# czbiohub-sf/biahub

Hardware: AMD Instinct MI355X
Metric: voxels/s for deskew+10-iter R-L deconv, 2048^2x512 f32 (higher is better)
Workload: dtype f32

## Files before the change

biahub_amd/build.py:

```python

from __future__ import annotations

import os
import subprocess
import sys
from concurrent.futures import ThreadPoolExecutor
from pathlib import Path

PKG = Path(__file__).resolve().parent
CSRC = PKG / "csrc"
INCLUDE = PKG.parent / "include"
LIB = PKG / "libbhcore.so"
SOURCES = ["pyramid.hip", "fftconv_col.hip", "fftconv_xtile.hip", "fftconv_xw.hip", "fftconv_colreg.hip", "deskew.hip", "stitch.hip", "stitch_pcc.hip", "affine.hip", "fftconv.hip", "context.hip", "fill.hip", "deconv.hip", "spline.hip", "copy.hip", "regmetric.hip", "flatfield.hip", "psf.hip", "binning.hip", "codec.hip", "lz4.hip", "zstd.hip", "mask.hip", "invtf.hip", "host_deskew.hip"]
ARCH = "gfx950"


def _hipcc() -> str:
    for cand in (os.environ.get("HIPCC"), "/opt/rocm/bin/hipcc", "hipcc"):
        if cand and (os.path.isabs(cand) and os.path.exists(cand) or not os.path.isabs(cand)):
            return cand
    return "hipcc"


_FC = ("fftconv.hpp", "fftconv_dev.hpp")
INCLUDES = {"fftconv.hip": _FC, "fftconv_col.hip": _FC, "fftconv_xtile.hip": _FC + ("fftconv_xpass.inc",), "fftconv_xw.hip": _FC + ("fftconv_xw.inc", "fftconv_x3.inc"),
            "fftconv_colreg.hip": _FC + ("fftconv_xw.inc", "fftconv_colw.inc", "fftconv_colz.inc", "fftconv_colz3.inc", "fftconv_zdirect.inc"),
            "deconv.hip": ("fftconv.hpp",), "invtf.hip": ("fftconv.hpp",), "affine.hip": ("affine_zwalk.inc", "affine_zoblique.inc"),
            "deskew.hip": ("deskew_geom.hpp", "deskew_rows.inc"), "host_deskew.hip": ("deskew_geom.hpp",), "zstd.hip": ("zstd_frame.inc", "zstd_block.inc")}


def needs_build() -> bool:
    if not LIB.exists():
        return True
    t = LIB.stat().st_mtime
    deps = [CSRC / s for s in SOURCES] + [CSRC / "common.hpp", INCLUDE / "bhcore.h"] + [CSRC / i for v in INCLUDES.values() for i in v]
    return any(d.stat().st_mtime > t for d in deps)


def build(force: bool = False, verbose: bool = True) -> Path:
    if not force and not needs_build():
        return LIB
    objdir = PKG / "build"
    objdir.mkdir(exist_ok=True)
    flags = ["-O3", f"--offload-arch={ARCH}", "-fPIC", "-std=c++17", f"-I{INCLUDE}", f"-I{CSRC}",
             "-Wall", "-Wno-unused-function"]

    def compile_one(src: str) -> Path:
# ... 26 lines not shown
```

biahub_amd/csrc/fftconv.hip:

```cpp
#include "fftconv_dev.hpp"

#include <mutex>

namespace bh {

static int x_tile_rows(int64_t X) { return X / 2 > 1024 ? 8 : BH_FC_XR; }

bool fftconv_supported_ex(int64_t Z, int64_t Y, int64_t X, bool radix3) {
    auto pow2 = [](int64_t v) { return v > 0 && (v & (v - 1)) == 0; };
    auto ok = [&](int64_t v) { return pow2(v) || (radix3 && ((v % 3 == 0 && pow2(v / 3)) || (v % 5 == 0 && pow2(v / 5)))); };
    if (!ok(Z) || !ok(Y) || !ok(X)) return false;
    if (X < 64 || X > 3072) return false;
    if (!pow2(X) && X / 2 / (X % 3 == 0 ? 3 : 5) < 32) return false;
    if (X / 4 > (X / 2 > 1024 ? BH_FC_XNT8 : BH_FC_XNT)) return false;
    if (Y < 2 * 16 || Y / 2 > 2048) return false;
    if (Z < 4 || Z > 2048) return false;
    const int xr = x_tile_rows(X);
    if ((Y % xr) != 0) return false;
    if (!pow2(Z) && Z / (Z % 3 == 0 ? 3 : 5) < 8) return false;
    if (!pow2(Y) && Y / 2 / (Y % 3 == 0 ? 3 : 5) < 16) return false;
    const int M = (int)X / 2, Lm = pow2(X) ? M : (X % 3 == 0 ? M / 3 : M / 5);
    const size_t xlds = (size_t)(M + 1) * (xr + 1) * 8 + (size_t)twiddle_count(Lm) * 8 + (size_t)M * 8 + (Lm != M ? (size_t)(M / Lm - 1) * Lm * 8 : 0);
    return xlds <= 160 * 1024;
}
// ... 301 lines not shown
    else
        hipLaunchKernelGGL(inverse_filter_rows_kernel<false>, dim3(grid), dim3(256), pl.d.XP * sizeof(cf), ctx->stream, tf, filt,
                           pl.d, reg, (float)(2.0 / V), bf16 ? 1 : 0, xcol);
    BH_CHECK_HIP(hipGetLastError());
    return BH_OK;
}

bool fftconv_fuses_normalisation(const ConvPlan& pl) { return pl.xw; }

int fftconv_apply_staged_filter(bh_ctx* ctx, const ConvPlan& pl, const float* in, const void* filt, bool bf16, cf* spec,
                                float* out, const double* norm_mean) {
    if (norm_mean) {
        BH_REQUIRE(pl.xw, "internal: fused normalisation needs the wave-private X passes");
        BH_TRY(launch_xw(ctx, pl, false, 0, in, spec, nullptr, nullptr, 0.f, false, norm_mean));
    } else
    BH_TRY(launch_x(ctx, pl, false, 0, in, spec, nullptr, nullptr, 0.f));
    BH_TRY(launch_col(ctx, pl, COL_FWD, false, spec, nullptr, 1.f));
    BH_TRY(launch_col(ctx, pl, bf16 ? COL_CONV16 : COL_CONV, true, spec, reinterpret_cast<const cf*>(filt), 1.f));
    BH_TRY(launch_col(ctx, pl, COL_INV, false, spec, nullptr, 1.f));
    BH_TRY(launch_x(ctx, pl, true, XE_STORE, nullptr, spec, out, nullptr, 0.f));
    return BH_OK;
}

int fftconv_richardson_lucy(bh_ctx* ctx, const ConvPlan& pl, const float* d, const cf* otf, bool otf_real, int zr, bool zreal, cf* spec,
                            int iterations, float eps, float* est) {
    if (iterations <= 0) return BH_OK;
    BH_TRY(launch_x(ctx, pl, false, 0, d, spec, est, nullptr, 0.f));
    for (int it = 0; it < iterations; ++it) {
        BH_TRY(launch_col(ctx, pl, COL_FWD, false, spec, nullptr, 1.f));
        BH_TRY(launch_rl_z(ctx, pl, false, otf_real, zr, zreal, spec, otf));
        BH_TRY(launch_col(ctx, pl, COL_INV, false, spec, nullptr, 1.f));
        BH_TRY(launch_x(ctx, pl, true, XE_RATIO, nullptr, spec, nullptr, d, eps, true));
        BH_TRY(launch_col(ctx, pl, COL_FWD, false, spec, nullptr, 1.f));
        BH_TRY(launch_rl_z(ctx, pl, true, otf_real, zr, zreal, spec, otf));
        BH_TRY(launch_col(ctx, pl, COL_INV, false, spec, nullptr, 1.f));
        BH_TRY(launch_x(ctx, pl, true, XE_UPDATE, nullptr, spec, est, est, eps, it + 1 < iterations));
    }
    return BH_OK;
}

int fftconv_tune_spectrum(bh_ctx* ctx, const ConvPlan& pl, float* est, size_t bytes, cf** spec) {
    const double V = (double)pl.d.Z * pl.d.Y * pl.d.X;
    const bool tune = env_int("BH_FC_TUNE_ALLOC", !(dev_alloc_is_shuffled() && dev_block_is_vmm(*spec))) != 0;
    if (!pl.xw || V < (double)(1u << 28) || !tune) return BH_OK;
    hipEvent_t e0, e1;
    BH_CHECK_HIP(hipEventCreate(&e0));
    BH_CHECK_HIP(hipEventCreate(&e1));
    auto audition = [&](cf* s, float* ms) -> int {
        for (int rep = 0; rep < 2; ++rep) {
            BH_CHECK_HIP(hipEventRecord(e0, ctx->stream));
            BH_TRY(launch_x(ctx, pl, true, XE_UPDATE, nullptr, s, est, est, 1e-6f, true));
            BH_CHECK_HIP(hipEventRecord(e1, ctx->stream));
            BH_CHECK_HIP(hipEventSynchronize(e1));
            BH_CHECK_HIP(hipEventElapsedTime(ms, e0, e1));
        }
        return BH_OK;
    };
    constexpr int NC = 5;
// ... 37 lines not shown
    BH_TRY(launch_col(ctx, pl, COL_FWD, false, spec, nullptr, 1.f));
    BH_TRY(launch_rl_z(ctx, pl, true, otf_real, zr, zreal, spec, otf));
    BH_TRY(launch_col(ctx, pl, COL_INV, false, spec, nullptr, 1.f));
    BH_TRY(launch_x(ctx, pl, true, XE_STORE, nullptr, spec, corr_p, nullptr, 0.f));
    return BH_OK;
}

bool fftconv_rl_wrap_supported(const ConvPlan& pl, const int64_t N[3], const int64_t K[3], const int64_t P[3]) {
    return pl.xw && N[1] == P[1] && K[2] <= 256 && getenv("BH_RL_NOWRAP") == nullptr;
}

int fftconv_richardson_lucy_wrap(bh_ctx* ctx, const ConvPlan& pl, const float* d_p, const cf* otf, bool otf_real, int zr, bool zreal, cf* spec_a,
                                 cf* spec_b, float* est_a, float* est_b, const int64_t N[3], const int64_t K[3], int iterations,
                                 float eps, float* out) {
    const int64_t P[3] = {pl.d.Z, pl.d.Y, pl.d.X};
    xw::Params::Wrap we[3], wr[3];
    for (int a = 0; a < 3; ++a) {
        const bool padded = P[a] != N[a];
        const int lo = padded ? (int)(K[a] - 1 - K[a] / 2) : 0, hi = padded ? (int)(K[a] / 2) : 0;
        we[a] = xw::Params::Wrap{(int)N[a], lo, lo, hi};
        wr[a] = xw::Params::Wrap{(int)N[a], lo, hi, lo};
    }
    float *cur = est_a, *nxt = est_b;
    BH_TRY(launch_x(ctx, pl, false, 0, d_p, spec_a, cur, nullptr, 0.f));
    for (int it = 0; it < iterations; ++it) {
        BH_TRY(launch_col(ctx, pl, COL_FWD, false, spec_a, nullptr, 1.f));
        BH_TRY(launch_rl_z(ctx, pl, false, otf_real, zr, zreal, spec_a, otf));
        BH_TRY(launch_col(ctx, pl, COL_INV, false, spec_a, nullptr, 1.f));
        BH_TRY(launch_xw_wrap(ctx, pl, xw::FUSED_RATIO_WRAP, spec_a, spec_b, nullptr, d_p, eps, wr[0], wr[2]));
        BH_TRY(launch_col(ctx, pl, COL_FWD, false, spec_b, nullptr, 1.f));
        BH_TRY(launch_rl_z(ctx, pl, true, otf_real, zr, zreal, spec_b, otf));
        BH_TRY(launch_col(ctx, pl, COL_INV, false, spec_b, nullptr, 1.f));
        if (it + 1 == iterations) {
            BH_TRY(launch_xw_wrap(ctx, pl, xw::INV_UPDATE_CROP, spec_b, nullptr, out, cur, eps, we[0], we[2]));
        } else {
            BH_TRY(launch_xw_wrap(ctx, pl, xw::FUSED_UPDATE_WRAP, spec_b, spec_a, nxt, cur, eps, we[0], we[2]));
            std::swap(cur, nxt);
        }
    }
    return BH_OK;
}

int fftconv_forward(bh_ctx* ctx, const ConvPlan& pl, const float* in, cf* spec) {
    BH_TRY(launch_x(ctx, pl, false, 0, in, spec, nullptr, nullptr, 0.f));
    BH_TRY(launch_col(ctx, pl, COL_FWD, false, spec, nullptr, 1.f));
    BH_TRY(launch_col(ctx, pl, COL_FWD, true, spec, nullptr, 1.f));
    return BH_OK;
}
int fftconv_inverse(bh_ctx* ctx, const ConvPlan& pl, cf* spec, float* out) {
    BH_TRY(launch_col(ctx, pl, COL_INV, true, spec, nullptr, 1.f));
    BH_TRY(launch_col(ctx, pl, COL_INV, false, spec, nullptr, 1.f));
    BH_TRY(launch_x(ctx, pl, true, XE_STORE, nullptr, spec, out, nullptr, 0.f));
    return BH_OK;
}

bool fftconv_pcc_peak_only(const ConvPlan& pl) { return pl.xw && !pl.x3 && getenv("BH_PCC_NO_FUSED_PEAK") == nullptr; }
int fftconv_pcc_apply(bh_ctx* ctx, const ConvPlan& pl, const float* img, cf* fixed, bool fixed_is_mov, bool roll, cf* s2, int norm,
// ... 33 lines not shown
```

biahub_amd/csrc/fftconv_colw.inc:

```
namespace colw {

#ifndef BH_COLW_NT
#define BH_COLW_NT 512
#endif
constexpr int NT = BH_COLW_NT;
constexpr int TILE_CF = 32 * NT;

template <int LOGN>
struct Geo {
    static constexpr int N = 1 << LOGN;
    static constexpr int W = TILE_CF / N;
    static constexpr int CPN = W / 2;
    static constexpr int N16 = N / 16, NQ = N / 256;
    static constexpr int LOWBITS = LOGN - 8;
    static constexpr int RC = 1 << LOWBITS;
    static constexpr int TILE_F4 = N * CPN + (N >> 5) * 8;
    static constexpr int NTA = 15 * N16, NTB = 15 * NQ;
    static constexpr size_t LDS_BYTES = (size_t)TILE_F4 * 16 + (size_t)(NTA + NTB) * 8;
};

template <int LOGN>
__host__ __device__ __forceinline__ constexpr int f4addr(int row, int cp) {
    return row * Geo<LOGN>::CPN + (row >> 5) * 8 + cp;
}

template <int LOGN>
__host__ __device__ __forceinline__ constexpr int row_a(int rest, int r) { return r * Geo<LOGN>::N16 + rest; }
template <int LOGN>
__host__ __device__ __forceinline__ constexpr int row_b(int rest, int r) {
// ... 93 lines not shown
    constexpr int DLOAD = LOAD_A ? 0 : DSPEC;
    constexpr int DSTORE = (MODE == COL_FWD || MODE == COL_FWD_SCALE) ? DSPEC : 0;
    extern __shared__ __attribute__((aligned(16))) unsigned char smem[];
    float4* tile = reinterpret_cast<float4*>(smem);
    cf* ta = reinterpret_cast<cf*>(smem + (size_t)G::TILE_F4 * 16);
    cf* tb = ta + G::NTA;
    const int tid = threadIdx.x;
    for (int i = tid; i < G::NTA + G::NTB; i += NT) ta[i] = p.tw[i];
    __syncthreads();
    const int cp = tid % G::CPN;
    const int ncoltiles = p.ncoltiles, nsub = p.nsub, XP = p.XP;
    const long outer_stride = p.outer_stride, sub_stride = p.sub_stride, row_stride = p.row_stride;
    const int ntiles = p.nouter * ncoltiles;
    auto tile_base = [=](int tt) -> long {
        const int ou = tt / ncoltiles;
        const int ct = tt - ou * ncoltiles;
        return (long)(ou / nsub) * outer_stride + (long)(ou % nsub) * sub_stride + (long)ct * G::W + 2 * cp;
    };
    const int rs = (int)row_stride;
    float4 pre[16];
    auto load_rows = [&](int tt, int rest) {
        const cf* src = p.S + tile_base(tt);
#pragma unroll
        for (int r = 0; r < 16; ++r) pre[r] = *reinterpret_cast<const float4*>(src + row_of<LOGN, DLOAD>(rest, r) * rs);
    };
    const int rest0 = tid / G::CPN;
    const int tstep = (int)gridDim.x;
    int t = (int)blockIdx.x;
    if (t < ntiles) load_rows(t, rest0);
    for (; t < ntiles; t += tstep) {
        const int rest = xw::opaque_i(rest0);
        const long base = tile_base(t);
        const int tn = t + tstep < ntiles ? t + tstep : t;
        cf x0[16], x1[16];
#pragma unroll
        for (int r = 0; r < 16; ++r) {
            x0[r] = make_float2(pre[r].x, pre[r].y);
            x1[r] = make_float2(pre[r].z, pre[r].w);
        }
        if (MODE == COL_INV) {
            load_rows(tn, rest);
            inverse<LOGN>(x0, x1, tile, ta, tb, rest, cp);
        } else if (!HAS_OTF) {
            load_rows(tn, rest);
            forward<LOGN>(x0, x1, tile, ta, tb, rest, cp);
            if (MODE == COL_FWD_SCALE) {
#pragma unroll
// ... 22 lines not shown
#pragma unroll
            for (int r = 0; r < 16; ++r) {
                const cf a0 = x0[r], a1 = x1[r];
                if (MODE == COL_FILTER) {
                    x0[r] = make_float2(a0.x * o[r].x, a0.y * o[r].y);
                    x1[r] = make_float2(a1.x * o[r].z, a1.y * o[r].w);
                } else if (MODE == COL_CORR) {
                    x0[r] = cmulc(a0, make_float2(o[r].x, o[r].y));
                    x1[r] = cmulc(a1, make_float2(o[r].z, o[r].w));
                } else {
                    x0[r] = cmul(a0, make_float2(o[r].x, o[r].y));
                    x1[r] = cmul(a1, make_float2(o[r].z, o[r].w));
                }
            }
            asm volatile("" ::: "memory");
            load_rows(tn, rest);
            __syncthreads();
            inverse<LOGN>(x0, x1, tile, ta, tb, rest, cp);
        }
        const bool col_ok = ((t % ncoltiles) * G::W + 2 * cp) < XP;
        if (col_ok) {
#pragma unroll
            for (int r = 0; r < 16; ++r)
                *reinterpret_cast<float4*>(p.S + base + row_of<LOGN, DSTORE>(rest, r) * rs) =
                    make_float4(x0[r].x, x0[r].y, x1[r].x, x1[r].y);
        }
        __syncthreads();
    }
}

template <int LOGN>
static void make_tables(std::vector<cf>& tab) {
    using G = Geo<LOGN>;
    tab.assign(G::NTA + G::NTB, make_float2(0.f, 0.f));
    for (int k = 1; k < 16; ++k) {
        for (int q = 0; q < G::N16; ++q) {
            const double a = -2.0 * M_PI * (double)q * k / (double)G::N;
            tab[(size_t)(k - 1) * G::N16 + q] = make_float2((float)std::cos(a), (float)std::sin(a));
        }
        for (int q = 0; q < G::NQ; ++q) {
            const double a = -2.0 * M_PI * (double)q * k / (double)G::N16;
            tab[G::NTA + (size_t)(k - 1) * G::NQ + q] = make_float2((float)std::cos(a), (float)std::sin(a));
        }
    }
}

}
```

biahub_amd/csrc/fftconv_dev.hpp:

```cpp
#pragma once
#include "fftconv.hpp"

#include <cmath>
#include <cstdio>
#include <cstdlib>
#include <utility>
#include <vector>

namespace bh {

#ifndef BH_FC_NT
#define BH_FC_NT 1024
#endif
constexpr int FC_NT = BH_FC_NT;
constexpr int FC_TILE = 16384;
#ifndef BH_FC_XR
#define BH_FC_XR 16
#endif
#ifndef BH_FC_XNT
#define BH_FC_XNT BH_FC_NT
#endif
#ifndef BH_FC_XNT8
#define BH_FC_XNT8 768
#endif
// ... 399 lines not shown
    float eps;
};

namespace xw {

enum Mode { FWD = 0, INV_STORE = 1, INV_RATIO = 2, INV_UPDATE = 3, FUSED_RATIO = 4, FUSED_UPDATE = 5, FUSED_RATIO_WRAP = 6, FUSED_UPDATE_WRAP = 7,
            INV_UPDATE_CROP = 8, INV_ARGMAX = 9 };

struct Params {
    const float* in;
    cf* S;
    float* out;
    const float* aux;
    const cf* tab;
    const cf* twy;
    int Z, Y, XP;
    float eps;
    const double* norm_mean;
    double* rowsum;
    cf* S_out;
    struct Wrap {
        int n, off, mlo, mhi;
    } wz, wx;
};

}


inline int ilog2(long v) {
    int l = 0;
    while ((1l << l) < v) ++l;
    return l;
}

inline bool env_off(const char* name) {
    const char* v = getenv(name);
    return v && atoi(v) == 0;
}
inline int env_int(const char* name, int dflt) {
    const char* v = getenv(name);
    return v ? atoi(v) : dflt;
}

template <typename K, typename P>
int launch_lds(bh_ctx* ctx, K kern, int grid, int threads, size_t lds, const P& p) {
    BH_CHECK_HIP(hipFuncSetAttribute(reinterpret_cast<const void*>(kern), hipFuncAttributeMaxDynamicSharedMemorySize, (int)lds));
    hipLaunchKernelGGL(kern, dim3(grid), dim3(threads), lds, ctx->stream, p);
    BH_CHECK_HIP(hipGetLastError());
    return BH_OK;
}

int launch_col_pass(bh_ctx* ctx, ColParams p, int mode);
int launch_col(bh_ctx* ctx, const ConvPlan& pl, int mode, bool zaxis, cf* S, const cf* otf, float scale, int pcc_norm = 0,
               int pcc_swap = 0, cf* otf_out = nullptr);
int launch_rl_z(bh_ctx* ctx, const ConvPlan& pl, bool corr, bool otf_real, int zr, bool zreal, cf* S, const cf* otf);
bool colw_tables(int64_t n, std::vector<cf>& tab);
bool colz_tables(const ConvDims& d, std::vector<cf>& tab);
bool colz3_tables(const ConvDims& d, std::vector<cf>& tab);
int launch_x_tile(bh_ctx* ctx, const ConvPlan& pl, bool inverse, int epi, const float* in, cf* S, float* out, const float* aux,
                  float eps, bool fuse_fwd);
void xw_tables(int64_t X, std::vector<cf>& tab, std::vector<int>& col);
int launch_xw(bh_ctx* ctx, const ConvPlan& pl, bool inverse, int epi, const float* in, cf* S, float* out, const float* aux,
              float eps, bool fuse_fwd, const double* norm_mean = nullptr);
int launch_xw_argmax(bh_ctx* ctx, const ConvPlan& pl, cf* S, ArgMax* partial, int* npartial);
int launch_xw_wrap(bh_ctx* ctx, const ConvPlan& pl, int mode, const cf* S_in, cf* S_out, float* out, const float* aux, float eps,
                   xw::Params::Wrap wz, xw::Params::Wrap wx);

}
```

biahub_amd/csrc/fftconv_xw.hip:

```cpp
#include "fftconv_dev.hpp"

namespace bh {

#include "fftconv_xw.inc"
#include "fftconv_x3.inc"

void xw_tables(int64_t X, std::vector<cf>& tab, std::vector<int>& col) {
    if (X == 3072) x3::make_tables<9>(tab, col);
    else if (X == 1536) x3::make_tables<8>(tab, col);
    else if (X == 2048) xw::make_tables<10>(tab, col);
    else if (X == 1024) xw::make_tables<9>(tab, col);
    else xw::make_tables<8>(tab, col);
}

template <int LOGM>
static int launch_xw_m(bh_ctx* ctx, const xw::Params& p, int mode, int* grid_out = nullptr) {
    using G = xw::Geo<LOGM>;
    const long npairs = (long)p.Z * (p.Y / 2);
    const int grid = (int)std::min<long>(ceil_div(npairs, (long)xw::NW * G::PAIRS), ctx->num_cus);
    if (grid_out) *grid_out = grid;
    auto run = [&](auto kern) { return launch_lds(ctx, kern, grid, xw::NT, G::LDS_BYTES, p); };
    switch (mode) {
        case xw::FWD: return run(xw::xw_kernel<LOGM, xw::FWD>);
        case xw::INV_STORE: return run(xw::xw_kernel<LOGM, xw::INV_STORE>);
// ... 8 lines not shown
    }
}

template <int LOGL>
static int launch_x3_m(bh_ctx* ctx, const xw::Params& p, int mode) {
    using G = x3::Geo<LOGL>;
    const long npairs = (long)p.Z * (p.Y / 2);
    const int grid = (int)std::min<long>(ceil_div(npairs, (long)x3::NW * G::PAIRS), ctx->num_cus);
    auto run = [&](auto kern) { return launch_lds(ctx, kern, grid, x3::NT, G::LDS_BYTES, p); };
    switch (mode) {
        case xw::FWD: return run(x3::x3_kernel<LOGL, xw::FWD>);
        case xw::INV_STORE: return run(x3::x3_kernel<LOGL, xw::INV_STORE>);
        case xw::INV_RATIO: return run(x3::x3_kernel<LOGL, xw::INV_RATIO>);
        case xw::INV_UPDATE: return run(x3::x3_kernel<LOGL, xw::INV_UPDATE>);
        case xw::FUSED_RATIO: return run(x3::x3_kernel<LOGL, xw::FUSED_RATIO>);
        case xw::FUSED_RATIO_WRAP: return run(x3::x3_kernel<LOGL, xw::FUSED_RATIO_WRAP>);
        case xw::FUSED_UPDATE_WRAP: return run(x3::x3_kernel<LOGL, xw::FUSED_UPDATE_WRAP>);
        case xw::INV_UPDATE_CROP: return run(x3::x3_kernel<LOGL, xw::INV_UPDATE_CROP>);
        default: return run(x3::x3_kernel<LOGL, xw::FUSED_UPDATE>);
    }
}

int launch_xw(bh_ctx* ctx, const ConvPlan& pl, bool inverse, int epi, const float* in, cf* S, float* out, const float* aux,
              float eps, bool fuse_fwd, const double* norm_mean) {
    xw::Params p;
    p.norm_mean = norm_mean;
    p.rowsum = nullptr;
    p.S_out = nullptr;
    p.wz = p.wx = xw::Params::Wrap{0, 0, 0, 0};
    p.in = in;
    p.S = S;
    p.out = out;
    p.aux = aux;
    p.tab = pl.xw_tab;
    p.twy = pl.twy;
    p.Z = pl.d.Z;
    p.Y = pl.d.Y;
    p.XP = pl.d.XP;
    p.eps = eps;
    const int mode = !inverse ? xw::FWD
                     : epi == XE_STORE ? xw::INV_STORE
                     : epi == XE_RATIO ? (fuse_fwd ? xw::FUSED_RATIO : xw::INV_RATIO)
                                       : (fuse_fwd ? xw::FUSED_UPDATE : xw::INV_UPDATE);
    if (mode == xw::INV_UPDATE && !pl.x3 && pl.rl_rowsums != nullptr) {
        p.rowsum = pl.rl_rowsums;
        const_cast<ConvPlan&>(pl).rl_rowsums_done = true;
    }
    if (pl.x3) return pl.d.M == 1536 ? launch_x3_m<9>(ctx, p, mode) : launch_x3_m<8>(ctx, p, mode);
    return pl.d.M == 1024 ? launch_xw_m<10>(ctx, p, mode) : (pl.d.M == 512 ? launch_xw_m<9>(ctx, p, mode) : launch_xw_m<8>(ctx, p, mode));
}

int launch_xw_argmax(bh_ctx* ctx, const ConvPlan& pl, cf* S, ArgMax* partial, int* npartial) {
    xw::Params p;
    p.norm_mean = nullptr;
    p.rowsum = nullptr;
    p.S_out = nullptr;
    p.wz = p.wx = xw::Params::Wrap{0, 0, 0, 0};
    p.in = nullptr;
    p.S = S;
    p.out = reinterpret_cast<float*>(partial);
    p.aux = nullptr;
    p.tab = pl.xw_tab;
    p.twy = pl.twy;
    p.Z = pl.d.Z;
    p.Y = pl.d.Y;
    p.XP = pl.d.XP;
    p.eps = 0.f;
    int grid = 0;
    BH_TRY(pl.d.M == 1024 ? launch_xw_m<10>(ctx, p, xw::INV_ARGMAX, &grid)
                          : (pl.d.M == 512 ? launch_xw_m<9>(ctx, p, xw::INV_ARGMAX, &grid) : launch_xw_m<8>(ctx, p, xw::INV_ARGMAX, &grid)));
    *npartial = grid * xw::NW;
    return BH_OK;
}

int launch_xw_wrap(bh_ctx* ctx, const ConvPlan& pl, int mode, const cf* S_in, cf* S_out, float* out, const float* aux, float eps,
                   xw::Params::Wrap wz, xw::Params::Wrap wx) {
    xw::Params p;
    p.norm_mean = nullptr;
    p.rowsum = nullptr;
    p.in = nullptr;
    p.S = const_cast<cf*>(S_in);
    p.S_out = S_out;
    p.out = out;
    p.aux = aux;
    p.tab = pl.xw_tab;
    p.twy = pl.twy;
    p.Z = pl.d.Z;
    p.Y = pl.d.Y;
    p.XP = pl.d.XP;
    p.eps = eps;
    p.wz = wz;
    p.wx = wx;
    if (!pl.x3) return pl.d.M == 1024 ? launch_xw_m<10>(ctx, p, mode) : (pl.d.M == 512 ? launch_xw_m<9>(ctx, p, mode) : launch_xw_m<8>(ctx, p, mode));
    return pl.d.M == 1536 ? launch_x3_m<9>(ctx, p, mode) : launch_x3_m<8>(ctx, p, mode);
}

}
```

biahub_amd/csrc/fftconv_xw.inc:

```
namespace xw {

constexpr int NT = 512;
constexpr int NW = NT / 64;

template <int LOGM>
struct Geo {
    static constexpr int M = 1 << LOGM;
    static constexpr int LG = M / 16;
    static constexpr int LOGLG = LOGM - 4;
    static constexpr int MIDBITS = LOGM - 6;
    static constexpr int R2 = 1 << MIDBITS;
    static constexpr int NREP = 16 / R2;
    static constexpr int BLK = M / 8;
    static constexpr int PADW = LOGM == 8 ? 0 : 8;
    static constexpr int BSTRIDE = BLK + PADW;
    static constexpr int ROWWORDS = 8 * BSTRIDE;
    static constexpr int PAIRS = 64 / LG;
    static constexpr int NTW1 = 7 * BLK, NTW2 = (R2 - 1) * 8, NUT = 8 * LG + 8;
    static constexpr int NTAB = NTW1 + NTW2 + NUT + (NTW2 & 1);
    static constexpr size_t LDS_BYTES = ((size_t)NTAB + (size_t)NW * PAIRS * 2 * ROWWORDS) * 8;
};

__host__ __device__ constexpr int parity(int v) {
    int p = 0;
    for (int b = 0; b < 16; ++b) p ^= (v >> b) & 1;
    return p;
// ... 492 lines not shown
        xb[i] = d;
    }
    nyA = make_float2(na + nb, 0.f);
    nyB = cmul(make_float2(na - nb, 0.f), wy);
}

__device__ __forceinline__ int opaque_i(int v) {
    asm volatile("" : "+v"(v));
    return v;
}

template <int LOGM, int MODE>
__global__ __launch_bounds__(NT) void xw_kernel(Params p) {
    using G = Geo<LOGM>;
    constexpr bool WRAP = MODE == FUSED_RATIO_WRAP || MODE == FUSED_UPDATE_WRAP;
    constexpr bool HAS_INV = MODE != FWD;
    constexpr bool HAS_FWD = MODE == FWD || MODE == FUSED_RATIO || MODE == FUSED_UPDATE || WRAP;
    constexpr bool RATIO = MODE == INV_RATIO || MODE == FUSED_RATIO || MODE == FUSED_RATIO_WRAP;
    constexpr bool CROP = MODE == INV_UPDATE_CROP;
    constexpr bool UPDATE = MODE == INV_UPDATE || MODE == FUSED_UPDATE || MODE == FUSED_UPDATE_WRAP || CROP;
    constexpr bool ARGMAX = MODE == INV_ARGMAX;
    constexpr bool STORE_REAL = MODE != FUSED_RATIO && MODE != FUSED_RATIO_WRAP && !ARGMAX;
    constexpr int M = G::M, LG = G::LG, X = 2 * M;
    extern __shared__ __attribute__((aligned(16))) unsigned char smem[];
    cf* tab = reinterpret_cast<cf*>(smem);
    const int tid = threadIdx.x;
    for (int i = tid; i < G::NTW1 + G::NTW2 + G::NUT; i += NT) tab[i] = p.tab[i];
    __syncthreads();
    const cf* tw1 = tab;
    const cf* tw2 = tab + G::NTW1;
    const cf* ut = tw2 + G::NTW2;
    const int wave = __builtin_amdgcn_readfirstlane(tid >> 6);
    const int lane = tid & 63;
    const int grp = lane / LG, l = lane % LG;
    unsigned char* ba = smem + (size_t)G::NTAB * 8 + (size_t)((wave * G::PAIRS + grp) * 2) * G::ROWWORDS * 8;
    const LaneAddr a0 = lane_addr<LOGM>(l);

    const int Yh = p.Y >> 1, XP = p.XP;
    const int npairs = p.Z * Yh;
    const int pstep = (int)gridDim.x * NW * G::PAIRS;
    const int laneS = grp * XP * 8 + l * 16;
    const int laneR = grp * X * 4 + l * 16;
    struct Rows {
        long ra, rb;
        long sa_, sb_;
        int yy;
// ... 14 lines not shown
            if (rel >= p.wz.n + p.wz.mhi) rel -= p.Z;
            r.zero = rel < -p.wz.mlo || rel >= p.wz.n + p.wz.mhi;
            rel += rel < 0 ? p.wz.n : (rel >= p.wz.n ? -p.wz.n : 0);
            const int zs = r.zero ? z : rel + p.wz.off;
            r.sa_ = (long)zs * p.Y + r.yy;
            r.sb_ = r.sa_ + Yh;
        }
        return r;
    };
    auto at = [](const void* base, long row, int pitch_bytes, int lane_off, int imm) {
        return reinterpret_cast<const float4*>(static_cast<const unsigned char*>(base) + row * pitch_bytes + (lane_off + imm));
    };
    auto at_w = [](void* base, long row, int pitch_bytes, int lane_off, int imm) {
        return reinterpret_cast<float4*>(static_cast<unsigned char*>(base) + row * pitch_bytes + (lane_off + imm));
    };

    float4 sa[8], sb[8];
    cf nya = make_float2(0.f, 0.f), nyb = nya;
    auto load_pair = [&](int pb) {
        const Rows r = rows_of(pb);
        if (HAS_INV) {
#pragma unroll
            for (int c = 0; c < 8; ++c) {
                sa[c] = *at(p.S, r.sa_, XP * 8, laneS, c * LG * 16);
                sb[c] = *at(p.S, r.sb_, XP * 8, laneS, c * LG * 16);
            }
            nya = *reinterpret_cast<const cf*>(reinterpret_cast<const unsigned char*>(p.S) + r.sa_ * XP * 8 + (grp * XP * 8 + M * 8));
            nyb = *reinterpret_cast<const cf*>(reinterpret_cast<const unsigned char*>(p.S) + r.sb_ * XP * 8 + (grp * XP * 8 + M * 8));
        } else {
#pragma unroll
            for (int c = 0; c < 8; ++c) {
                sa[c] = *at(p.in, r.ra, X * 4, laneR, c * (G::BLK / 2) * 16);
                sb[c] = *at(p.in, r.rb, X * 4, laneR, c * (G::BLK / 2) * 16);
            }
        }
    };

    float best_v = -1.0f;
    long best_i = 0;
    int pb = (blockIdx.x * NW + wave) * G::PAIRS;
    if (pb < npairs) load_pair(pb);
    for (; pb < npairs; pb += pstep) {
        LaneAddr a = a0;
        a.dr_c4 = opaque_i(a.dr_c4);
        a.d2_c4 = opaque_i(a.d2_c4);
        a.d3_c4[0] = opaque_i(a.d3_c4[0]);
        a.d3_c4[1] = opaque_i(a.d3_c4[1]);
        const Rows rw = rows_of(pb);
        const cf wy = p.twy[rw.yy + grp];
        const int pnext = pb + pstep < npairs ? pb + pstep : pb;
        cf xa[16], xb[16];
#pragma unroll
        for (int c = 0; c < 8; ++c) {
            xa[2 * c] = make_float2(sa[c].x, sa[c].y);
            xa[2 * c + 1] = make_float2(sa[c].z, sa[c].w);
            xb[2 * c] = make_float2(sb[c].x, sb[c].y);
            xb[2 * c + 1] = make_float2(sb[c].z, sb[c].w);
        }
        if (HAS_INV) {
            const cf nya_cur = nya, nyb_cur = nyb;
            if (MODE == INV_STORE || ARGMAX) load_pair(pnext);
            float4 auxa[8], auxb[8];
            auto load_aux_a = [&]() {
#pragma unroll
                for (int r = 0; r < 8; ++r) auxa[r] = *at(p.aux, rw.sa_, X * 4, laneR, r * (G::BLK / 2) * 16);
            };
            auto load_aux_b = [&]() {
#pragma unroll
                for (int r = 0; r < 8; ++r) auxb[r] = *at(p.aux, rw.sb_, X * 4, laneR, r * (G::BLK / 2) * 16);
            };
            pair_inv_head<LOGM>(xa, xb, nya_cur, nyb_cur, wy, ba, tw2, ut, l, a);
            if (RATIO || UPDATE) {
                load_aux_a();
                load_aux_b();
            }
            const bool zero_plane = rw.zero;
            auto tail_row = [&](cf (&x)[16], const float4 (&aux)[8], const unsigned char* buf, long row) {
                const int zq = CROP ? (int)(row / p.Y) - p.wz.off : 0;
                const long yq = CROP ? row % p.Y + grp : 0;
                get_dr<LOGM>(buf, x, a);
                xw_fence();
                stage_top1<LOGM, true>(x, tw1, l);
                xw_fence();
#pragma unroll
                for (int r = 0; r < 8; ++r) {
                    float4 v = pack2(x[2 * r], x[2 * r + 1]);
                    if (RATIO) {
                        v.x = aux[r].x / fmaxf(v.x, p.eps);
                        v.y = aux[r].y / fmaxf(v.y, p.eps);
                        v.z = aux[r].z / fmaxf(v.z, p.eps);
                        v.w = aux[r].w / fmaxf(v.w, p.eps);
                    } else if (UPDATE) {
                        v.x = fmaxf(aux[r].x * v.x, 0.0f);
                        v.y = fmaxf(aux[r].y * v.y, 0.0f);
                        v.z = fmaxf(aux[r].z * v.z, 0.0f);
                        v.w = fmaxf(aux[r].w * v.w, 0.0f);
                    }
                    if (ARGMAX) {
                        const float ax = fabsf(v.x), ay = fabsf(v.y), az = fabsf(v.z), aw = fabsf(v.w);
                        const float m = fmaxf(fmaxf(ax, ay), fmaxf(az, aw));
                        if (m >= best_v) {
                            const int e = ax == m ? 0 : (ay == m ? 1 : (az == m ? 2 : 3));
                            const long i = (row + grp) * X + (2 * r * G::BLK + 4 * l + e);
                            if (m > best_v || i < best_i) {
                                best_v = m;
                                best_i = i;
                            }
                        }
                    }
                    if (CROP) {
                        const int xq = 2 * r * G::BLK + 4 * l - p.wx.off;
                        if (zq >= 0 && zq < p.wz.n) {
                            float* dst = p.out + ((long)zq * p.Y + yq) * p.wx.n + xq;
                            typedef float f4u __attribute__((ext_vector_type(4), aligned(4)));
                            if (xq >= 0 && xq + 3 < p.wx.n) {
                                *reinterpret_cast<f4u*>(dst) = f4u{v.x, v.y, v.z, v.w};
                            } else {
                                const float v4[4] = {v.x, v.y, v.z, v.w};
#pragma unroll
                                for (int e = 0; e < 4; ++e)
                                    if (xq + e >= 0 && xq + e < p.wx.n) dst[e] = v4[e];
                            }
                        }
                    } else if (STORE_REAL && !WRAP) *at_w(p.out, row, X * 4, laneR, r * (G::BLK / 2) * 16) = v;
                    x[2 * r] = make_float2(v.x, v.y);
                    x[2 * r + 1] = make_float2(v.z, v.w);
                }
                if (MODE == INV_UPDATE && p.rowsum != nullptr) {
                    double sd = 0.0;
#pragma unroll
                    for (int r = 0; r < 8; ++r)
                        sd += ((double)x[2 * r].x + (double)x[2 * r].y) + ((double)x[2 * r + 1].x + (double)x[2 * r + 1].y);
#pragma unroll
                    for (int o = LG / 2; o > 0; o >>= 1) sd += __shfl_xor(sd, o, 64);
                    if (l == 0) p.rowsum[row + grp] = sd;
                }
                if (WRAP) {
                    const int n = p.wx.n, off = p.wx.off, mlo = p.wx.mlo, mhi = p.wx.mhi;
                    float* scr = reinterpret_cast<float*>(const_cast<unsigned char*>(buf));
#pragma unroll
                    for (int r = 0; r < 8; ++r) {
                        const int n0 = 2 * r * G::BLK - off, n1 = n0 + 2 * G::BLK;
                        if ((n1 > n - mlo && n0 < n) || (n0 < mhi && n1 > 0)) {
                            const float v4[4] = {x[2 * r].x, x[2 * r].y, x[2 * r + 1].x, x[2 * r + 1].y};
#pragma unroll
                            for (int e = 0; e < 4; ++e) {
                                const int nn = n0 + 4 * l + e;
// ... 7 lines not shown
                    for (int r = 0; r < 8; ++r) {
                        const int n0 = 2 * r * G::BLK - off, n1 = n0 + 2 * G::BLK;
                        if (n0 < 0 || n1 > n) {
                            float v4[4] = {x[2 * r].x, x[2 * r].y, x[2 * r + 1].x, x[2 * r + 1].y};
#pragma unroll
                            for (int e = 0; e < 4; ++e) {
                                int rel = n0 + 4 * l + e;
                                if (rel >= n + mhi) rel -= X;
                                const bool inside = rel >= 0 && rel < n, low = rel >= -mlo && rel < 0, high = rel >= n && rel < n + mhi;
                                const float m = scr[low ? rel + mlo : (high ? mlo + rel - n : 0)];
                                v4[e] = inside ? v4[e] : ((low || high) ? m : 0.0f);
                            }
                            x[2 * r] = make_float2(v4[0], v4[1]);
                            x[2 * r + 1] = make_float2(v4[2], v4[3]);
                        }
                    }
                    if (zero_plane) {
#pragma unroll
                        for (int i = 0; i < 16; ++i) x[i] = make_float2(0.f, 0.f);
                    }
                    xw_fence();
                    if (STORE_REAL) {
#pragma unroll
                        for (int r = 0; r < 8; ++r) *at_w(p.out, row, X * 4, laneR, r * (G::BLK / 2) * 16) = pack2(x[2 * r], x[2 * r + 1]);
                    }
                }
                xw_fence();
            };
            tail_row(xa, auxa, ba, rw.ra);
            tail_row(xb, auxb, ba + G::ROWWORDS * 8, rw.rb);
            if (MODE == INV_RATIO || MODE == INV_UPDATE || CROP) load_pair(pnext);
        } else if (p.norm_mean) {
            const float inv = (float)(1.0 / *p.norm_mean);
#pragma unroll
            for (int i = 0; i < 16; ++i) {
                xa[i] = make_float2(xa[i].x * inv - 1.0f, xa[i].y * inv - 1.0f);
                xb[i] = make_float2(xb[i].x * inv - 1.0f, xb[i].y * inv - 1.0f);
            }
        } else if (p.out) {
#pragma unroll
            for (int r = 0; r < 8; ++r) {
                xa[2 * r] = make_float2(fmaxf(xa[2 * r].x, 0.f), fmaxf(xa[2 * r].y, 0.f));
                xa[2 * r + 1] = make_float2(fmaxf(xa[2 * r + 1].x, 0.f), fmaxf(xa[2 * r + 1].y, 0.f));
                xb[2 * r] = make_float2(fmaxf(xb[2 * r].x, 0.f), fmaxf(xb[2 * r].y, 0.f));
                xb[2 * r + 1] = make_float2(fmaxf(xb[2 * r + 1].x, 0.f), fmaxf(xb[2 * r + 1].y, 0.f));
                *at_w(p.out, rw.ra, X * 4, laneR, r * (G::BLK / 2) * 16) = pack2(xa[2 * r], xa[2 * r + 1]);
                *at_w(p.out, rw.rb, X * 4, laneR, r * (G::BLK / 2) * 16) = pack2(xb[2 * r], xb[2 * r + 1]);
            }
        }
        if (HAS_FWD) {
            xw_fence();
            load_pair(pnext);
            xw_fence();
            transform_fwd<LOGM>(xa, xb, ba, tw1, tw2, l, a);
            cf nyA, nyB;
            pair_fwd_tail<LOGM>(xa, xb, nyA, nyB, wy, ut, l);
#pragma unroll
            for (int c = 0; c < 8; ++c) {
                *at_w(Sdst, rw.ra, XP * 8, laneS, c * LG * 16) = pack2(xa[2 * c], xa[2 * c + 1]);
                *at_w(Sdst, rw.rb, XP * 8, laneS, c * LG * 16) = pack2(xb[2 * c], xb[2 * c + 1]);
            }
            if (l < 16) {
                const cf zero = make_float2(0.f, 0.f);
                unsigned char* S8 = reinterpret_cast<unsigned char*>(Sdst);
                const int off = grp * XP * 8 + (M + l) * 8;
                *reinterpret_cast<cf*>(S8 + rw.ra * XP * 8 + off) = l == 0 ? nyA : zero;
                *reinterpret_cast<cf*>(S8 + rw.rb * XP * 8 + off) = l == 0 ? nyB : zero;
            }
        }
    }
    if (ARGMAX) {
#pragma unroll
        for (int o = 32; o > 0; o >>= 1) {
            const float ov = __shfl_xor(best_v, o);
            const long oi = ((long)__shfl_xor((int)(best_i >> 32), o) << 32) | (unsigned int)__shfl_xor((int)best_i, o);
            if (ov > best_v || (ov == best_v && oi < best_i)) {
                best_v = ov;
                best_i = oi;
            }
        }
        if (lane == 0) reinterpret_cast<ArgMax*>(p.out)[blockIdx.x * NW + wave] = ArgMax{best_v, (long long)best_i};
    }
}
// ... 27 lines not shown
```

Measured before the change: 6.986 billion.

## Skip first R-L estimate store and use nontemporal loads/stores in FFT passes

The first Richardson-Lucy forward X pass no longer writes the clamped estimate to memory. The first update pass instead reads the raw data with a clamp-to-zero flag, which removes one full-volume write and the matching read. Separately, the wave-private X passes and the column passes now use nontemporal loads and stores for their streaming spectrum and real-plane traffic, to reduce cache pollution. The nontemporal hints could hurt if any of those buffers are reused soon after from cache.

```diff
diff --git a/biahub_amd/build.py b/biahub_amd/build.py
--- a/biahub_amd/build.py
+++ b/biahub_amd/build.py
@@ -22,7 +22,7 @@
     return "hipcc"
 
 
-_FC = ("fftconv.hpp", "fftconv_dev.hpp")
+_FC = ("fftconv.hpp", "fftconv_dev.hpp", "stream_once.hpp")
 INCLUDES = {"fftconv.hip": _FC, "fftconv_col.hip": _FC, "fftconv_xtile.hip": _FC + ("fftconv_xpass.inc",), "fftconv_xw.hip": _FC + ("fftconv_xw.inc", "fftconv_x3.inc"),
             "fftconv_colreg.hip": _FC + ("fftconv_xw.inc", "fftconv_colw.inc", "fftconv_colz.inc", "fftconv_colz3.inc", "fftconv_zdirect.inc"),
             "deconv.hip": ("fftconv.hpp",), "invtf.hip": ("fftconv.hpp",), "affine.hip": ("affine_zwalk.inc", "affine_zoblique.inc"),
diff --git a/biahub_amd/csrc/fftconv.hip b/biahub_amd/csrc/fftconv.hip
--- a/biahub_amd/csrc/fftconv.hip
+++ b/biahub_amd/csrc/fftconv.hip
@@ -347,9 +347,14 @@
     return BH_OK;
 }
 
+static bool rl_skips_first_estimate(const ConvPlan& pl) { return pl.xw && !pl.x3 && env_int("BH_RL_FIRST_EST_STORE", 0) == 0; }
+
 int fftconv_richardson_lucy(bh_ctx* ctx, const ConvPlan& pl, const float* d, const cf* otf, bool otf_real, int zr, bool zreal, cf* spec,
                             int iterations, float eps, float* est) {
     if (iterations <= 0) return BH_OK;
+    const bool skip0 = rl_skips_first_estimate(pl);
+    if (skip0) BH_TRY(launch_xw(ctx, pl, false, 0, d, spec, nullptr, nullptr, 0.f, false, nullptr, true));
+    else
     BH_TRY(launch_x(ctx, pl, false, 0, d, spec, est, nullptr, 0.f));
     for (int it = 0; it < iterations; ++it) {
         BH_TRY(launch_col(ctx, pl, COL_FWD, false, spec, nullptr, 1.f));
@@ -359,6 +364,8 @@
         BH_TRY(launch_col(ctx, pl, COL_FWD, false, spec, nullptr, 1.f));
         BH_TRY(launch_rl_z(ctx, pl, true, otf_real, zr, zreal, spec, otf));
         BH_TRY(launch_col(ctx, pl, COL_INV, false, spec, nullptr, 1.f));
+        if (skip0 && it == 0) BH_TRY(launch_xw(ctx, pl, true, XE_UPDATE, nullptr, spec, est, d, eps, it + 1 < iterations, nullptr, true));
+        else
         BH_TRY(launch_x(ctx, pl, true, XE_UPDATE, nullptr, spec, est, est, eps, it + 1 < iterations));
     }
     return BH_OK;
@@ -442,6 +449,9 @@
         wr[a] = xw::Params::Wrap{(int)N[a], lo, hi, lo};
     }
     float *cur = est_a, *nxt = est_b;
+    const bool skip0 = rl_skips_first_estimate(pl);
+    if (skip0) BH_TRY(launch_xw(ctx, pl, false, 0, d_p, spec_a, nullptr, nullptr, 0.f, false, nullptr, true));
+    else
     BH_TRY(launch_x(ctx, pl, false, 0, d_p, spec_a, cur, nullptr, 0.f));
     for (int it = 0; it < iterations; ++it) {
         BH_TRY(launch_col(ctx, pl, COL_FWD, false, spec_a, nullptr, 1.f));
@@ -451,8 +461,12 @@
         BH_TRY(launch_col(ctx, pl, COL_FWD, false, spec_b, nullptr, 1.f));
         BH_TRY(launch_rl_z(ctx, pl, true, otf_real, zr, zreal, spec_b, otf));
         BH_TRY(launch_col(ctx, pl, COL_INV, false, spec_b, nullptr, 1.f));
+        const bool first = skip0 && it == 0;
+        const float* operand = first ? d_p : cur;
         if (it + 1 == iterations) {
-            BH_TRY(launch_xw_wrap(ctx, pl, xw::INV_UPDATE_CROP, spec_b, nullptr, out, cur, eps, we[0], we[2]));
+            BH_TRY(launch_xw_wrap(ctx, pl, xw::INV_UPDATE_CROP, spec_b, nullptr, out, operand, eps, we[0], we[2], first));
+        } else if (first) {
+            BH_TRY(launch_xw_wrap(ctx, pl, xw::FUSED_UPDATE_WRAP, spec_b, spec_a, cur, operand, eps, we[0], we[2], true));
         } else {
             BH_TRY(launch_xw_wrap(ctx, pl, xw::FUSED_UPDATE_WRAP, spec_b, spec_a, nxt, cur, eps, we[0], we[2]));
             std::swap(cur, nxt);
diff --git a/biahub_amd/csrc/fftconv_colw.inc b/biahub_amd/csrc/fftconv_colw.inc
--- a/biahub_amd/csrc/fftconv_colw.inc
+++ b/biahub_amd/csrc/fftconv_colw.inc
@@ -5,6 +5,13 @@
 #endif
 constexpr int NT = BH_COLW_NT;
 constexpr int TILE_CF = 32 * NT;
+
+#ifndef BH_NT_COLW_LD
+#define BH_NT_COLW_LD 1
+#endif
+#ifndef BH_NT_COLW_ST
+#define BH_NT_COLW_ST 1
+#endif
 
 template <int LOGN>
 struct Geo {
@@ -144,7 +151,7 @@
     auto load_rows = [&](int tt, int rest) {
         const cf* src = p.S + tile_base(tt);
 #pragma unroll
-        for (int r = 0; r < 16; ++r) pre[r] = *reinterpret_cast<const float4*>(src + row_of<LOGN, DLOAD>(rest, r) * rs);
+        for (int r = 0; r < 16; ++r) pre[r] = ld_once<BH_NT_COLW_LD>(reinterpret_cast<const float4*>(src + row_of<LOGN, DLOAD>(rest, r) * rs));
     };
     const int rest0 = tid / G::CPN;
     const int tstep = (int)gridDim.x;
@@ -213,8 +220,8 @@
         if (col_ok) {
 #pragma unroll
             for (int r = 0; r < 16; ++r)
-                *reinterpret_cast<float4*>(p.S + base + row_of<LOGN, DSTORE>(rest, r) * rs) =
-                    make_float4(x0[r].x, x0[r].y, x1[r].x, x1[r].y);
+                st_once<BH_NT_COLW_ST>(reinterpret_cast<float4*>(p.S + base + row_of<LOGN, DSTORE>(rest, r) * rs),
+                                       make_float4(x0[r].x, x0[r].y, x1[r].x, x1[r].y));
         }
         __syncthreads();
     }
diff --git a/biahub_amd/csrc/fftconv_dev.hpp b/biahub_amd/csrc/fftconv_dev.hpp
--- a/biahub_amd/csrc/fftconv_dev.hpp
+++ b/biahub_amd/csrc/fftconv_dev.hpp
@@ -1,5 +1,6 @@
 #pragma once
 #include "fftconv.hpp"
+#include "stream_once.hpp"
 
 #include <cmath>
 #include <cstdio>
@@ -445,6 +446,7 @@
     struct Wrap {
         int n, off, mlo, mhi;
     } wz, wx;
+    int clamp0;
 };
 
 }
@@ -484,9 +486,9 @@
                   float eps, bool fuse_fwd);
 void xw_tables(int64_t X, std::vector<cf>& tab, std::vector<int>& col);
 int launch_xw(bh_ctx* ctx, const ConvPlan& pl, bool inverse, int epi, const float* in, cf* S, float* out, const float* aux,
-              float eps, bool fuse_fwd, const double* norm_mean = nullptr);
+              float eps, bool fuse_fwd, const double* norm_mean = nullptr, bool clamp0 = false);
 int launch_xw_argmax(bh_ctx* ctx, const ConvPlan& pl, cf* S, ArgMax* partial, int* npartial);
 int launch_xw_wrap(bh_ctx* ctx, const ConvPlan& pl, int mode, const cf* S_in, cf* S_out, float* out, const float* aux, float eps,
-                   xw::Params::Wrap wz, xw::Params::Wrap wx);
-
-}
+                   xw::Params::Wrap wz, xw::Params::Wrap wx, bool clamp0 = false);
+
+}
diff --git a/biahub_amd/csrc/fftconv_xw.hip b/biahub_amd/csrc/fftconv_xw.hip
--- a/biahub_amd/csrc/fftconv_xw.hip
+++ b/biahub_amd/csrc/fftconv_xw.hip
@@ -54,8 +54,9 @@
 }
 
 int launch_xw(bh_ctx* ctx, const ConvPlan& pl, bool inverse, int epi, const float* in, cf* S, float* out, const float* aux,
-              float eps, bool fuse_fwd, const double* norm_mean) {
+              float eps, bool fuse_fwd, const double* norm_mean, bool clamp0) {
     xw::Params p;
+    p.clamp0 = clamp0;
     p.norm_mean = norm_mean;
     p.rowsum = nullptr;
     p.S_out = nullptr;
@@ -78,12 +79,17 @@
         p.rowsum = pl.rl_rowsums;
         const_cast<ConvPlan&>(pl).rl_rowsums_done = true;
     }
-    if (pl.x3) return pl.d.M == 1536 ? launch_x3_m<9>(ctx, p, mode) : launch_x3_m<8>(ctx, p, mode);
-    return pl.d.M == 1024 ? launch_xw_m<10>(ctx, p, mode) : (pl.d.M == 512 ? launch_xw_m<9>(ctx, p, mode) : launch_xw_m<8>(ctx, p, mode));
+    if (pl.x3) {
+        BH_REQUIRE(!clamp0, "internal: the radix-3 X passes store their first estimate");
+        return pl.d.M == 1536 ? launch_x3_m<9>(ctx, p, mode) : launch_x3_m<8>(ctx, p, mode);
+    }
+    return pl.d.M == 1024 ? launch_xw_m<10>(ctx, p, mode)
+                          : (pl.d.M == 512 ? launch_xw_m<9>(ctx, p, mode) : launch_xw_m<8>(ctx, p, mode));
 }
 
 int launch_xw_argmax(bh_ctx* ctx, const ConvPlan& pl, cf* S, ArgMax* partial, int* npartial) {
     xw::Params p;
+    p.clamp0 = 0;
     p.norm_mean = nullptr;
     p.rowsum = nullptr;
     p.S_out = nullptr;
@@ -106,8 +112,9 @@
 }
 
 int launch_xw_wrap(bh_ctx* ctx, const ConvPlan& pl, int mode, const cf* S_in, cf* S_out, float* out, const float* aux, float eps,
-                   xw::Params::Wrap wz, xw::Params::Wrap wx) {
+                   xw::Params::Wrap wz, xw::Params::Wrap wx, bool clamp0) {
     xw::Params p;
+    p.clamp0 = clamp0;
     p.norm_mean = nullptr;
     p.rowsum = nullptr;
     p.in = nullptr;
@@ -123,7 +130,10 @@
     p.eps = eps;
     p.wz = wz;
     p.wx = wx;
-    if (!pl.x3) return pl.d.M == 1024 ? launch_xw_m<10>(ctx, p, mode) : (pl.d.M == 512 ? launch_xw_m<9>(ctx, p, mode) : launch_xw_m<8>(ctx, p, mode));
+    if (!pl.x3)
+        return pl.d.M == 1024 ? launch_xw_m<10>(ctx, p, mode)
+                              : (pl.d.M == 512 ? launch_xw_m<9>(ctx, p, mode) : launch_xw_m<8>(ctx, p, mode));
+    BH_REQUIRE(!clamp0, "internal: the radix-3 X passes store their first estimate");
     return pl.d.M == 1536 ? launch_x3_m<9>(ctx, p, mode) : launch_x3_m<8>(ctx, p, mode);
 }
 
diff --git a/biahub_amd/csrc/fftconv_xw.inc b/biahub_amd/csrc/fftconv_xw.inc
--- a/biahub_amd/csrc/fftconv_xw.inc
+++ b/biahub_amd/csrc/fftconv_xw.inc
@@ -2,6 +2,19 @@
 
 constexpr int NT = 512;
 constexpr int NW = NT / 64;
+
+#ifndef BH_NT_XW_LD
+#define BH_NT_XW_LD 1
+#endif
+#ifndef BH_NT_XW_AUX
+#define BH_NT_XW_AUX 1
+#endif
+#ifndef BH_NT_XW_ST_REAL
+#define BH_NT_XW_ST_REAL 1
+#endif
+#ifndef BH_NT_XW_ST_SPEC
+#define BH_NT_XW_ST_SPEC 1
+#endif
 
 template <int LOGM>
 struct Geo {
@@ -540,6 +553,7 @@
     constexpr bool ARGMAX = MODE == INV_ARGMAX;
     constexpr bool STORE_REAL = MODE != FUSED_RATIO && MODE != FUSED_RATIO_WRAP && !ARGMAX;
     constexpr int M = G::M, LG = G::LG, X = 2 * M;
+    constexpr bool NT_LD = BH_NT_XW_LD && !WRAP, NT_AUX = BH_NT_XW_AUX && !WRAP && UPDATE, NT_REAL = BH_NT_XW_ST_REAL, NT_SPEC = BH_NT_XW_ST_SPEC;
     extern __shared__ __attribute__((aligned(16))) unsigned char smem[];
     cf* tab = reinterpret_cast<cf*>(smem);
     const int tid = threadIdx.x;
@@ -600,20 +614,21 @@
         if (HAS_INV) {
 #pragma unroll
             for (int c = 0; c < 8; ++c) {
-                sa[c] = *at(p.S, r.sa_, XP * 8, laneS, c * LG * 16);
-                sb[c] = *at(p.S, r.sb_, XP * 8, laneS, c * LG * 16);
+                sa[c] = ld_once<NT_LD>(at(p.S, r.sa_, XP * 8, laneS, c * LG * 16));
+                sb[c] = ld_once<NT_LD>(at(p.S, r.sb_, XP * 8, laneS, c * LG * 16));
             }
             nya = *reinterpret_cast<const cf*>(reinterpret_cast<const unsigned char*>(p.S) + r.sa_ * XP * 8 + (grp * XP * 8 + M * 8));
             nyb = *reinterpret_cast<const cf*>(reinterpret_cast<const unsigned char*>(p.S) + r.sb_ * XP * 8 + (grp * XP * 8 + M * 8));
         } else {
 #pragma unroll
             for (int c = 0; c < 8; ++c) {
-                sa[c] = *at(p.in, r.ra, X * 4, laneR, c * (G::BLK / 2) * 16);
-                sb[c] = *at(p.in, r.rb, X * 4, laneR, c * (G::BLK / 2) * 16);
+                sa[c] = ld_once<NT_LD>(at(p.in, r.ra, X * 4, laneR, c * (G::BLK / 2) * 16));
+                sb[c] = ld_once<NT_LD>(at(p.in, r.rb, X * 4, laneR, c * (G::BLK / 2) * 16));
             }
         }
     };
 
+    const float aux_lo = p.clamp0 ? 0.0f : -__builtin_huge_valf();
     float best_v = -1.0f;
     long best_i = 0;
     int pb = (blockIdx.x * NW + wave) * G::PAIRS;
@@ -641,11 +656,11 @@
             float4 auxa[8], auxb[8];
             auto load_aux_a = [&]() {
 #pragma unroll
-                for (int r = 0; r < 8; ++r) auxa[r] = *at(p.aux, rw.sa_, X * 4, laneR, r * (G::BLK / 2) * 16);
+                for (int r = 0; r < 8; ++r) auxa[r] = ld_once<NT_AUX>(at(p.aux, rw.sa_, X * 4, laneR, r * (G::BLK / 2) * 16));
             };
             auto load_aux_b = [&]() {
 #pragma unroll
-                for (int r = 0; r < 8; ++r) auxb[r] = *at(p.aux, rw.sb_, X * 4, laneR, r * (G::BLK / 2) * 16);
+                for (int r = 0; r < 8; ++r) auxb[r] = ld_once<NT_AUX>(at(p.aux, rw.sb_, X * 4, laneR, r * (G::BLK / 2) * 16));
             };
             pair_inv_head<LOGM>(xa, xb, nya_cur, nyb_cur, wy, ba, tw2, ut, l, a);
             if (RATIO || UPDATE) {
@@ -669,10 +684,15 @@
                         v.z = aux[r].z / fmaxf(v.z, p.eps);
                         v.w = aux[r].w / fmaxf(v.w, p.eps);
                     } else if (UPDATE) {
-                        v.x = fmaxf(aux[r].x * v.x, 0.0f);
-                        v.y = fmaxf(aux[r].y * v.y, 0.0f);
-                        v.z = fmaxf(aux[r].z * v.z, 0.0f);
-                        v.w = fmaxf(aux[r].w * v.w, 0.0f);
+                        float4 e = aux[r];
+                        e.x = fmaxf(e.x, aux_lo);
+                        e.y = fmaxf(e.y, aux_lo);
+                        e.z = fmaxf(e.z, aux_lo);
+                        e.w = fmaxf(e.w, aux_lo);
+                        v.x = fmaxf(e.x * v.x, 0.0f);
+                        v.y = fmaxf(e.y * v.y, 0.0f);
+                        v.z = fmaxf(e.z * v.z, 0.0f);
+                        v.w = fmaxf(e.w * v.w, 0.0f);
                     }
                     if (ARGMAX) {
                         const float ax = fabsf(v.x), ay = fabsf(v.y), az = fabsf(v.z), aw = fabsf(v.w);
@@ -700,7 +720,7 @@
                                     if (xq + e >= 0 && xq + e < p.wx.n) dst[e] = v4[e];
                             }
                         }
-                    } else if (STORE_REAL && !WRAP) *at_w(p.out, row, X * 4, laneR, r * (G::BLK / 2) * 16) = v;
+                    } else if (STORE_REAL && !WRAP) st_once<NT_REAL>(at_w(p.out, row, X * 4, laneR, r * (G::BLK / 2) * 16), v);
                     x[2 * r] = make_float2(v.x, v.y);
                     x[2 * r + 1] = make_float2(v.z, v.w);
                 }
@@ -754,7 +774,7 @@
                     xw_fence();
                     if (STORE_REAL) {
 #pragma unroll
-                        for (int r = 0; r < 8; ++r) *at_w(p.out, row, X * 4, laneR, r * (G::BLK / 2) * 16) = pack2(x[2 * r], x[2 * r + 1]);
+                        for (int r = 0; r < 8; ++r) st_once<NT_REAL>(at_w(p.out, row, X * 4, laneR, r * (G::BLK / 2) * 16), pack2(x[2 * r], x[2 * r + 1]));
                     }
                 }
                 xw_fence();
@@ -769,15 +789,17 @@
                 xa[i] = make_float2(xa[i].x * inv - 1.0f, xa[i].y * inv - 1.0f);
                 xb[i] = make_float2(xb[i].x * inv - 1.0f, xb[i].y * inv - 1.0f);
             }
-        } else if (p.out) {
+        } else if (p.out || p.clamp0) {
 #pragma unroll
             for (int r = 0; r < 8; ++r) {
                 xa[2 * r] = make_float2(fmaxf(xa[2 * r].x, 0.f), fmaxf(xa[2 * r].y, 0.f));
                 xa[2 * r + 1] = make_float2(fmaxf(xa[2 * r + 1].x, 0.f), fmaxf(xa[2 * r + 1].y, 0.f));
                 xb[2 * r] = make_float2(fmaxf(xb[2 * r].x, 0.f), fmaxf(xb[2 * r].y, 0.f));
                 xb[2 * r + 1] = make_float2(fmaxf(xb[2 * r + 1].x, 0.f), fmaxf(xb[2 * r + 1].y, 0.f));
-                *at_w(p.out, rw.ra, X * 4, laneR, r * (G::BLK / 2) * 16) = pack2(xa[2 * r], xa[2 * r + 1]);
-                *at_w(p.out, rw.rb, X * 4, laneR, r * (G::BLK / 2) * 16) = pack2(xb[2 * r], xb[2 * r + 1]);
+                if (p.out) {
+                    *at_w(p.out, rw.ra, X * 4, laneR, r * (G::BLK / 2) * 16) = pack2(xa[2 * r], xa[2 * r + 1]);
+                    *at_w(p.out, rw.rb, X * 4, laneR, r * (G::BLK / 2) * 16) = pack2(xb[2 * r], xb[2 * r + 1]);
+                }
             }
         }
         if (HAS_FWD) {
@@ -789,8 +811,8 @@
             pair_fwd_tail<LOGM>(xa, xb, nyA, nyB, wy, ut, l);
 #pragma unroll
             for (int c = 0; c < 8; ++c) {
-                *at_w(Sdst, rw.ra, XP * 8, laneS, c * LG * 16) = pack2(xa[2 * c], xa[2 * c + 1]);
-                *at_w(Sdst, rw.rb, XP * 8, laneS, c * LG * 16) = pack2(xb[2 * c], xb[2 * c + 1]);
+                st_once<NT_SPEC>(at_w(Sdst, rw.ra, XP * 8, laneS, c * LG * 16), pack2(xa[2 * c], xa[2 * c + 1]));
+                st_once<NT_SPEC>(at_w(Sdst, rw.rb, XP * 8, laneS, c * LG * 16), pack2(xb[2 * c], xb[2 * c + 1]));
             }
             if (l < 16) {
                 const cf zero = make_float2(0.f, 0.f);
diff --git a/biahub_amd/csrc/stream_once.hpp b/biahub_amd/csrc/stream_once.hpp
--- /dev/null
+++ b/biahub_amd/csrc/stream_once.hpp
@@ -0,0 +1,38 @@
+#pragma once
+#include <hip/hip_runtime.h>
+
+namespace bh {
+
+typedef float so_f4 __attribute__((ext_vector_type(4)));
+typedef float so_f2 __attribute__((ext_vector_type(2)));
+
+template <bool NT>
+__device__ __forceinline__ float4 ld_once(const float4* p) {
+    if constexpr (NT) {
+        const so_f4 v = __builtin_nontemporal_load(reinterpret_cast<const so_f4*>(p));
+        return make_float4(v.x, v.y, v.z, v.w);
+    } else {
+        return *p;
+    }
+}
+template <bool NT>
+__device__ __forceinline__ float2 ld_once(const float2* p) {
+    if constexpr (NT) {
+        const so_f2 v = __builtin_nontemporal_load(reinterpret_cast<const so_f2*>(p));
+        return make_float2(v.x, v.y);
+    } else {
+        return *p;
+    }
+}
+template <bool NT>
+__device__ __forceinline__ void st_once(float4* p, float4 v) {
+    if constexpr (NT) __builtin_nontemporal_store(so_f4{v.x, v.y, v.z, v.w}, reinterpret_cast<so_f4*>(p));
+    else *p = v;
+}
+template <bool NT>
+__device__ __forceinline__ void st_once(float2* p, float2 v) {
+    if constexpr (NT) __builtin_nontemporal_store(so_f2{v.x, v.y}, reinterpret_cast<so_f2*>(p));
+    else *p = v;
+}
+
+}
```

Result: slower. 6.862 billion (-1.8%).
